# ZHANGKEON/DIS-YOLO

Hardware: AMD Instinct MI355X
Metric: train images/sec @576x576 bf16 (higher is better)
Workload: dtype bf16

## Files before the change

### dis-yolo_amd/csrc/conv_wgrad.hip

```cpp
#include "common.h"
#include "runtime.h"

namespace {

struct WgradParams {
  const bf16* x0;
  const bf16* x1;
  const bf16* dy;
  float* out;
  int B, H, W, C0, C1, Cin;
  int Ho, Wo, Cout, ldy;
  int ks, stride, pad_t, pad_l;
  int M, K;
  int steps_per_split, steps;
  int tilesK, tilesN;
  unsigned bytes0, bytes1, bytesy;
};

typedef __attribute__((address_space(3))) s16x4 lds_s16x4;
typedef int i32x4 __attribute__((ext_vector_type(4)));
constexpr unsigned OOB = 0x80000000u;

__device__ __forceinline__ int swz_u(int row, int u, int units) {
  const int h = (row & 3) | (((row >> 3) & 1) << 2);
// ... 93 lines not shown
#pragma unroll
  for (int j = 0; j < YI; ++j) {
    const int chunk = (j * NW + wave) * 64 + lane;
    const int row = chunk / YCH, pc = chunk % YCH;
    const int lc = swz_u(row, pc >> 1, YCH / 2) * 2 + (pc & 1);
    const int n = n0 + lc * 8;
    y_nok[j] = (row < 32) && (n < p.ldy);
    y_m[j] = step0 * 32 + row;
    y_off[j] = ((unsigned)y_m[j] * (unsigned)p.ldy + (unsigned)n) * 2u;
  }

  const bool mixed = (p.C1 > 0) && ((p.C0 & (BM - 1)) != 0);
  const bool blk_second = (p.C1 > 0) && (kt0 >= p.C0);
  auto issue_tile = [&](int stage) {
    const unsigned sbase = lds0 + stage * STB + wave * 1024;
#pragma unroll
    for (int j = 0; j < XI; ++j) {
      const int iy = x_yo[j] * p.stride - p.pad_t + x_kh[j];
      const int ix = x_xo[j] * p.stride - p.pad_l + x_kw[j];
      const bool ok = x_kok[j] && (x_b[j] < p.B) && ((unsigned)iy < (unsigned)p.H) && ((unsigned)ix < (unsigned)p.W);
      unsigned off;
      if (!x_second[j]) {
        off = (unsigned)(((x_b[j] * p.H + iy) * p.W + ix) * p.C0 + x_ci[j]) * 2u;
      } else {
        const int H1 = p.H >> 1, W1 = p.W >> 1;
        off = (unsigned)(((x_b[j] * H1 + (iy >> 1)) * W1 + (ix >> 1)) * p.C1 + x_ci[j]) * 2u;
      }
      if (!mixed) {
        if (blk_second) dma16(ok ? off : OOB, srd1, sbase + j * SLAB);
        else dma16(ok ? off : OOB, srd0, sbase + j * SLAB);
      } else {
        const void* src = ok ? (const void*)((const char*)(x_second[j] ? p.x1 : p.x0) + off) : (const void*)&g_zero16;
        dma16_flat(src, sbase + j * SLAB);
      }
      x_xo[j] += 32;
      while (x_xo[j] >= p.Wo) {
        x_xo[j] -= p.Wo;
        if (++x_yo[j] == p.Ho) {
          x_yo[j] = 0;
          ++x_b[j];
        }
      }
    }
#pragma unroll
    for (int j = 0; j < YI; ++j) {
      dma16((y_nok[j] && y_m[j] < p.M) ? y_off[j] : OOB, srdy, sbase + X_BYTES + j * SLAB);
      y_m[j] += 32;
      y_off[j] += 32u * (unsigned)p.ldy * 2u;
    }
  };

  f32x4 acc[MI][NI];
#pragma unroll
  for (int i = 0; i < MI; ++i)
#pragma unroll
    for (int j = 0; j < NI; ++j) acc[i][j] = f32x4{0.f, 0.f, 0.f, 0.f};

#pragma unroll
  for (int s = 0; s < PRE; ++s)
    if (s < nsteps) issue_tile(s);

  const int g = lane >> 4, li = lane & 15, q = li >> 2, pc = li & 3;
  for (int st = 0; st < nsteps; ++st) {
    if (PRE >= 1 && st + PRE - 1 < nsteps)
      wait_vmcnt<LPT*(PRE >= 1 ? PRE - 1 : 0)>();
    else
      wait_vmcnt<0>();
    __builtin_amdgcn_s_barrier();
    asm volatile("" ::: "memory");
    if (st + PRE < nsteps) issue_tile((st + PRE) % ST);
    const char* sX = smem + (st % ST) * STB;
    const char* sY = sX + X_BYTES;
    bf16x8 af[MI], bfr[NI];
    typedef short s16x8 __attribute__((ext_vector_type(8)));
    const int r0 = 8 * g + q, r1 = r0 + 4;
#pragma unroll
    for (int i = 0; i < MI; ++i) {
      const int u = (wm * WTM + i * 16) >> 4;
      const s16x4 lo = __builtin_amdgcn_ds_read_tr16_b64_v4i16(
          (lds_s16x4*)(sX + r0 * XP + swz_u(r0, u, XCH / 2) * 32 + pc * 8));
      const s16x4 hi = __builtin_amdgcn_ds_read_tr16_b64_v4i16(
          (lds_s16x4*)(sX + r1 * XP + swz_u(r1, u, XCH / 2) * 32 + pc * 8));
      const s16x8 v = {lo[0], lo[1], lo[2], lo[3], hi[0], hi[1], hi[2], hi[3]};
      af[i] = __builtin_bit_cast(bf16x8, v);
    }
#pragma unroll
    for (int j = 0; j < NI; ++j) {
      const int u = (wn * WTN + j * 16) >> 4;
      const s16x4 lo = __builtin_amdgcn_ds_read_tr16_b64_v4i16(
          (lds_s16x4*)(sY + r0 * YP + swz_u(r0, u, YCH / 2) * 32 + pc * 8));
      const s16x4 hi = __builtin_amdgcn_ds_read_tr16_b64_v4i16(
          (lds_s16x4*)(sY + r1 * YP + swz_u(r1, u, YCH / 2) * 32 + pc * 8));
      const s16x8 v = {lo[0], lo[1], lo[2], lo[3], hi[0], hi[1], hi[2], hi[3]};
      bfr[j] = __builtin_bit_cast(bf16x8, v);
    }
#pragma unroll
    for (int i = 0; i < MI; ++i)
#pragma unroll
      for (int j = 0; j < NI; ++j)
        acc[i][j] = __builtin_amdgcn_mfma_f32_16x16x32_bf16(af[i], bfr[j], acc[i][j], 0, 0, 0);
  }

  float* slab = p.out + (size_t)bsplit * p.K * p.Cout;
  __syncthreads();
  constexpr int ROWP = WTN * 4 + 16;
  constexpr int HALF = MI / 2 * 16;
  if constexpr (NW * HALF * ROWP <= ST * STB) {
    if ((p.Cout & 3) == 0) {
      char* sw = smem + wave * (HALF * ROWP);
      constexpr int CPR4 = WTN / 4, CH = HALF * CPR4;
#pragma unroll
      for (int h = 0; h < 2; ++h) {
#pragma unroll
        for (int i2 = 0; i2 < MI / 2; ++i2)
#pragma unroll
          for (int j = 0; j < NI; ++j)
#pragma unroll
            for (int r = 0; r < 4; ++r)
              *reinterpret_cast<float*>(sw + (i2 * 16 + g * 4 + r) * ROWP + (j * 16 + li) * 4) = acc[h * (MI / 2) + i2][j][r];
        __builtin_amdgcn_fence(__ATOMIC_RELEASE, "wavefront");
        __builtin_amdgcn_wave_barrier();
        __builtin_amdgcn_fence(__ATOMIC_ACQUIRE, "wavefront");
#pragma unroll
        for (int it = 0; it < (CH + 63) / 64; ++it) {
          const int idx = it * 64 + lane;
          const int row = idx / CPR4, ch = idx % CPR4;
          const int kk = kt0 + wm * WTM + h * HALF + row, n = n0 + wn * WTN + ch * 4;
          if (idx < CH && kk < p.K && n < p.Cout)
            *reinterpret_cast<float4*>(slab + (size_t)kk * p.Cout + n) =
                *reinterpret_cast<const float4*>(sw + row * ROWP + ch * 16);
        }
        __builtin_amdgcn_fence(__ATOMIC_RELEASE, "wavefront");
        __builtin_amdgcn_wave_barrier();
      }
      return;
    }
  }
#pragma unroll
  for (int i = 0; i < MI; ++i) {
#pragma unroll
    for (int j = 0; j < NI; ++j) {
      const int n = n0 + wn * WTN + j * 16 + li;
      if (n >= p.Cout) continue;
#pragma unroll
      for (int r = 0; r < 4; ++r) {
        const int kk = kt0 + wm * WTM + i * 16 + g * 4 + r;
        if (kk < p.K) slab[(size_t)kk * p.Cout + n] = acc[i][j][r];
      }
    }
  }
}


struct Wg3Params {
  const bf16* x;
  const bf16* dy;
  float* out;
  int B, H, W, Cin, Cout, ldy;
  int Ho, Wo;
  int P, Hp, frame, kbias;
  int a64, r64;
  int chunks, chunks_per_split;
  int tilesCi, tilesCo, tiles;
  int leadA, leadB;
  unsigned bytesx, bytesy;
  int debug;
};

struct PixState {
  int b, yy, xx;
};
__device__ __forceinline__ void pix_init(PixState& s, int Q, const Wg3Params& p) {
  const int Qn = Q + p.kbias * p.frame;
  const int bb = Qn / p.frame;
  const int rem = Qn - bb * p.frame;
  s.b = bb - p.kbias;
  s.yy = rem / p.P;
  s.xx = rem - s.yy * p.P;
}
__device__ __forceinline__ void pix_advance64(PixState& s, const Wg3Params& p) {
  s.xx += p.r64;
  s.yy += p.a64;
  if (s.xx >= p.P) {
    s.xx -= p.P;
    ++s.yy;
  }
  while (s.yy >= p.Hp) {
    s.yy -= p.Hp;
    ++s.b;
  }
}
__device__ __forceinline__ int pix_index(const PixState& s, const Wg3Params& p) {
  const bool ok = ((unsigned)s.b < (unsigned)p.B) && (s.yy >= 1) && (s.xx >= 1);
  return ok ? (s.b * p.H + s.yy - 1) * p.W + s.xx - 1 : -1;
}

__device__ __forceinline__ int pix_index_s2_in(const PixState& s, const Wg3Params& p) {
  const bool ok = ((unsigned)s.b < (unsigned)p.B) && (s.yy < p.Ho) && (s.xx < p.Wo);
  return ok ? (s.b * p.H + 2 * s.yy) * p.W + 2 * s.xx : -1;
}
__device__ __forceinline__ int pix_index_s2_out(const PixState& s, const Wg3Params& p) {
  const bool ok = ((unsigned)s.b < (unsigned)p.B) && (s.yy < p.Ho) && (s.xx < p.Wo);
  return ok ? (s.b * p.Ho + s.yy) * p.Wo + s.xx : -1;
}

template <int IMM>
__device__ __forceinline__ void dma16_imm(unsigned voff, i32x4 srd, unsigned lds_dst) {
  asm volatile("s_mov_b32 m0, %2\n\ts_nop 0\n\tbuffer_load_dwordx4 %0, %1, 0 offen offset:%3 lds"
               :
               : "v"(voff), "s"(srd), "s"(lds_dst - (unsigned)IMM), "n"(IMM)
               : "memory");
}

template <int CO_T, int R, int ST, int NW, int S2 = 0>
__global__ __launch_bounds__(NW * 64) void conv_wgrad3x3_kernel(Wg3Params p) {
  constexpr int NJ = CO_T / 32;
  constexpr int YD = CO_T / 32;
  constexpr int YDW = YD * 4 / NW;
  constexpr int TPW = NW == 8 ? 5 : 9;
  constexpr int YST = YD * 4096;
  constexpr int XRING = R * 4096;
  constexpr int XALLOC = XRING + 1024;
  constexpr int NR = S2 ? 4 : 1;
  constexpr int XTOT = NR * XALLOC;
  constexpr int PRE = ST - 1;
  constexpr int LPT0 = NR + YDW, LPT1 = YDW;
  static_assert(!S2 || NW == 4, "stride 2: the four-wave form only");
  static_assert((R & (R - 1)) == 0 && ST >= 2, "ring");

  extern __shared__ __attribute__((aligned(16))) char smem[];
  const unsigned lds0 = (unsigned)(size_t)(__attribute__((address_space(3))) char*)smem;
  const int tid = threadIdx.x, lane = tid & 63;
  const int wave = __builtin_amdgcn_readfirstlane(tid >> 6);
  const int wq = wave & 3, tg = wave >> 2;
  const int u = wq & 1, ch = wq >> 1;
  const int tap0 = tg * 5, ntaps = NW == 8 ? (tg ? 4 : 5) : 9;
  int lin;
  {
    const int nblk = gridDim.x, bid = blockIdx.x;
    const int q8 = nblk >> 3, r8 = nblk & 7, xcd = bid & 7, loc = bid >> 3;
    lin = (xcd < r8 ? xcd * (q8 + 1) : r8 * (q8 + 1) + (xcd - r8) * q8) + loc;
  }
  const int tile = lin % p.tiles, bsplit = lin / p.tiles;
  const int ci0 = (tile % p.tilesCi) * 32, co0 = (tile / p.tilesCi) * CO_T;
  const int c0 = bsplit * p.chunks_per_split;
  int c1 = c0 + p.chunks_per_split;
  if (c1 > p.chunks) c1 = p.chunks;
  const int nsteps = c1 - c0;

  const i32x4 srdx = make_srd(p.x, p.bytesx);
  const i32x4 srdy = make_srd(p.dy, p.bytesy);

  const int drow = wq * 16 + (lane >> 2), dpc = lane & 3;
  const int dlu = (dpc >> 1) ^ ((drow >> 2) & 1);
  const unsigned x_const = (unsigned)(ci0 + dlu * 16 + (dpc & 1) * 8) * 2u;
  const int y_n = co0 + (NW == 8 ? tg * 32 : 0) + dlu * 16 + (dpc & 1) * 8;
  const unsigned y_const = (unsigned)y_n * 2u;
  PixState xs, ys;
  pix_init(xs, (c0 - p.leadB) * 64 + drow, p);
  pix_init(ys, c0 * 64 + drow, p);
  const unsigned xrow_bytes = (unsigned)p.Cin * 2u, yrow_bytes = (unsigned)p.ldy * 2u;
  auto issue_x = [&](int c) {
    const unsigned slot = (unsigned)(c & (R - 1));
    if constexpr (S2) {
      const int pix = pix_index_s2_in(xs, p);
#pragma unroll
      for (int cls = 0; cls < 4; ++cls) {
        const unsigned voff = pix >= 0 ? (unsigned)(pix + (cls >> 1) * p.W + (cls & 1)) * xrow_bytes + x_const : OOB;
        if (wave == 0 && slot == 0) dma16(voff, srdx, lds0 + cls * XALLOC + XRING);
        dma16(voff, srdx, lds0 + cls * XALLOC + slot * 4096u + wq * 1024u);
      }
    } else {
      const int pix = pix_index(xs, p);
      const unsigned voff = pix >= 0 ? (unsigned)pix * xrow_bytes + x_const : OOB;
      if (tg == 0) {
        if (wave == 0 && slot == 0) dma16(voff, srdx, lds0 + XRING);
        dma16(voff, srdx, lds0 + slot * 4096u + wq * 1024u);
      }
    }
    pix_advance64(xs, p);
  };
  auto issue_y = [&](int stage) {
    const int pix = S2 ? pix_index_s2_out(ys, p) : pix_index(ys, p);
    const unsigned voff = pix >= 0 ? (unsigned)pix * yrow_bytes + y_const : OOB;
    const unsigned dst = lds0 + XTOT + stage * YST + (NW == 8 ? tg * 4096u : 0u) + wq * 1024u;
    dma16_imm<0>((y_n < p.ldy) ? voff : OOB, srdy, dst);
    if constexpr (NW == 4) {
      dma16_imm<64>((y_n + 32 < p.ldy) ? voff : OOB, srdy, dst + 4096u);
      if constexpr (YD == 4) {
        dma16_imm<128>((y_n + 64 < p.ldy) ? voff : OOB, srdy, dst + 8192u);
        dma16_imm<192>((y_n + 96 < p.ldy) ? voff : OOB, srdy, dst + 12288u);
      }
    } else if constexpr (YD == 4) {
      dma16_imm<128>((y_n + 64 < p.ldy) ? voff : OOB, srdy, dst + 8192u);
    }
    pix_advance64(ys, p);
  };

  const int g = lane >> 4, li = lane & 15, q = li >> 2, pc = li & 3;
  int E[TPW], EC[TPW];
#pragma unroll
  for (int i = 0; i < TPW; ++i) {
    const int tap = tap0 + i;
    const int kh = tap / 3, kw = tap % 3;
    const int rowc = (S2 ? (kh >> 1) * p.P + (kw >> 1) : (kh - 1) * p.P + (kw - 1)) + 4 * g + q;
    E[i] = rowc * 64 + ((u ^ ((rowc >> 2) & 1)) * 32) + pc * 8;
// ... 150 lines not shown
  const unsigned gbase = (unsigned)grp * 2u * F1_STB;
  const int g = lane >> 4, li = lane & 15, q = li >> 2, pc = li & 3;
  const i32x4 srdy = make_srd(dy, bytesy);
  const int drow = wave * 16 + (lane >> 2), dpc = lane & 3;
  const unsigned y_const = (unsigned)((((dpc >> 1) ^ ((drow >> 2) & 1)) * 16 + (dpc & 1) * 8) * 2);
  int e_x[2], e_c[2];
#pragma unroll
  for (int h = 0; h < 2; ++h) {
    const int e = tid + h * 256;
    e_x[h] = e / 3;
    e_c[h] = e - e_x[h] * 3;
  }
  float iv[3][2];
  auto unit_of = [&](int u, int& b, int& y, int& x0) {
    const int xb = u % units_x, r = u / units_x;
    y = r % H;
    b = r / H;
    x0 = xb * 128;
  };
  auto issue_dy = [&](int stage, int b, int y, int x0) {
#pragma unroll
    for (int s2 = 0; s2 < 2; ++s2) {
      const int x = x0 + s2 * 64 + drow;
      const unsigned voff = x < W ? (unsigned)((b * H + y) * W + x) * 64u + y_const : OOB;
      dma16(voff, srdy, lds0 + gbase + stage * F1_STB + F1_IMGB + s2 * 4096 + wave * 1024);
    }
  };
  auto load_img = [&](int b, int y, int x0) {
#pragma unroll
    for (int kh = 0; kh < 3; ++kh) {
      const int yy = y + kh - 1;
#pragma unroll
      for (int h = 0; h < 2; ++h) {
        const int x = x0 - 1 + e_x[h];
        const bool ok = (tid + h * 256 < 390) && ((unsigned)yy < (unsigned)H) && ((unsigned)x < (unsigned)W);
        iv[kh][h] = ok ? img[((size_t)(b * H + yy) * W + x) * 3 + e_c[h]] : 0.f;
      }
    }
  };
  auto write_img = [&](int stage) {
    char* base = smem + gbase + stage * F1_STB;
#pragma unroll
    for (int kh = 0; kh < 3; ++kh)
#pragma unroll
      for (int h = 0; h < 2; ++h) {
        if (tid + h * 256 >= 390) continue;
        const bf16 v = (bf16)iv[kh][h];
#pragma unroll
        for (int kw = 0; kw < 3; ++kw) {
          const int j = e_x[h] - kw;
          if ((unsigned)j < 128u) *reinterpret_cast<bf16*>(base + ((kh * 3 + kw) * 3 + e_c[h]) * F1_ROWB + j * 2) = v;
        }
      }
  };
  f32x4 acc[2][2];
#pragma unroll
  for (int f = 0; f < 2; ++f)
#pragma unroll
    for (int j = 0; j < 2; ++j) acc[f][j] = f32x4{0.f, 0.f, 0.f, 0.f};
  const int a_off = li * F1_ROWB + (32 * wave + 4 * g) * 2;
  const bool a1_ok = 16 + li < 27;
  const int brow = 4 * g + q;
  int Fy[2];
#pragma unroll
  for (int j = 0; j < 2; ++j)
    Fy[j] = F1_IMGB + (wave >> 1) * 4096 + (wave & 1) * 2048 + brow * 64 + ((j ^ ((brow >> 2) & 1)) * 32) + pc * 8;

  int u = blockIdx.x * 2 + grp;
  const int ustep = gridDim.x * 2;
  int stage = 0;
  if (u < nunits) {
    int b, y, x0;
    unit_of(u, b, y, x0);
    issue_dy(0, b, y, x0);
    load_img(b, y, x0);
    write_img(0);
  }
  wait_vmcnt<0>();
  __syncthreads();
  typedef short s16x8 __attribute__((ext_vector_type(8)));
  const int rounds = (nunits - (int)blockIdx.x * 2 + ustep - 1) / ustep;
  for (int it = 0; it < rounds; ++it, u += ustep) {
    const int un = u + ustep;
    const bool more = un < nunits;
    if (more) {
      int b, y, x0;
      unit_of(un, b, y, x0);
      issue_dy(stage ^ 1, b, y, x0);
      load_img(b, y, x0);
    }
    const char* sb = smem + gbase + stage * F1_STB;
    if (u < nunits) {
    bf16x8 af[2], bfr[2];
    {
      const uint2 lo = *reinterpret_cast<const uint2*>(sb + a_off), hi = *reinterpret_cast<const uint2*>(sb + a_off + 32);
      const uint4 v = {lo.x, lo.y, hi.x, hi.y};
      af[0] = __builtin_bit_cast(bf16x8, v);
      uint4 w = {0u, 0u, 0u, 0u};
      if (a1_ok) {
        const uint2 lo1 = *reinterpret_cast<const uint2*>(sb + a_off + 16 * F1_ROWB);
        const uint2 hi1 = *reinterpret_cast<const uint2*>(sb + a_off + 16 * F1_ROWB + 32);
        w = uint4{lo1.x, lo1.y, hi1.x, hi1.y};
      }
      af[1] = __builtin_bit_cast(bf16x8, w);
    }
#pragma unroll
    for (int j = 0; j < 2; ++j) {
      const char* a = sb + Fy[j];
      const s16x4 lo = __builtin_amdgcn_ds_read_tr16_b64_v4i16((lds_s16x4*)a);
      const s16x4 hi = __builtin_amdgcn_ds_read_tr16_b64_v4i16((lds_s16x4*)(a + 1024));
      const s16x8 v = {lo[0], lo[1], lo[2], lo[3], hi[0], hi[1], hi[2], hi[3]};
      bfr[j] = __builtin_bit_cast(bf16x8, v);
    }
#pragma unroll
    for (int f = 0; f < 2; ++f)
#pragma unroll
      for (int j = 0; j < 2; ++j) acc[f][j] = __builtin_amdgcn_mfma_f32_16x16x32_bf16(af[f], bfr[j], acc[f][j], 0, 0, 0);
    }
    if (more) write_img(stage ^ 1);
    wait_vmcnt<0>();
    __syncthreads();
    stage ^= 1;
  }
  float* red = reinterpret_cast<float*>(smem);
  __syncthreads();
#pragma unroll
  for (int f = 0; f < 2; ++f)
#pragma unroll
    for (int j = 0; j < 2; ++j)
#pragma unroll
      for (int r = 0; r < 4; ++r) red[((grp * 4 + wave) * 32 + 16 * f + 4 * g + r) * 32 + 16 * j + li] = acc[f][j][r];
  __syncthreads();
  float* slab = slabs + (size_t)blockIdx.x * 27 * 32;
  for (int o = threadIdx.x; o < 27 * 32; o += 512)
    slab[o] = ((red[o] + red[1024 + o]) + (red[2048 + o] + red[3072 + o])) + ((red[4096 + o] + red[5120 + o]) + (red[6144 + o] + red[7168 + o]));
}

void plan(const disyolo_conv_desc* d, int* bn, int* splits, int* steps_per_split, int* steps) {
  const int M = d->B * d->Ho * d->Wo;
  const int K = d->ksize * d->ksize * (d->C0 + d->C1);
  *bn = d->Cout > 64 ? 128 : (d->Cout > 32 ? 64 : 32);
  const int tiles = ceil_div(K, 128) * ceil_div(d->Cout, *bn);
  *steps = ceil_div(M, 32);
  const int target = 256, min_steps = 16;
  int s = target / tiles;
  if (s < 1) s = 1;
  const int max_s = ceil_div(*steps, min_steps);
  if (s > max_s) s = max_s;
  if (s < 1) s = 1;
  *steps_per_split = ceil_div(*steps, s);
  *splits = ceil_div(*steps, *steps_per_split);
}


constexpr int WG3_ST = 3;
struct Plan3 {
  int co_t, R, splits, cps, chunks, tilesCi, tilesCo, leadA, leadB, s2;
  size_t lds;
};
bool plan3(const disyolo_conv_desc* d, int opts, Plan3* q) {
  const int target = 192;
  if (opts & DISYOLO_WGRAD_IM2COL) return false;
  if (d->ksize != 3 || d->C1 != 0 || d->in_div != 1 || d->C0 % 32 || d->Cout % 4 || d->Cout < 32) return false;
  q->s2 = 0;
  if (d->stride == 2) {
    if (d->pad_t != 0 || d->pad_l != 0 || (d->H & 1) || (d->W & 1) || d->Ho * 2 != d->H || d->Wo * 2 != d->W) return false;
    q->s2 = 1;
  } else if (d->stride != 1 || d->pad_t != 1 || d->pad_l != 1 || d->Ho != d->H || d->Wo != d->W) {
    return false;
  }
  const int P = d->Wo + 1, Hp = d->Ho + 1;
  q->co_t = d->Cout > 64 ? 128 : 64;
  if (q->co_t == 128) {
    const int t128 = (d->C0 / 32) * ceil_div(d->Cout, 128);
    if ((target + t128 / 2) / t128 == 2) q->co_t = 64;
  }
  q->leadB = q->s2 ? 0 : ceil_div(P + 1, 64);
  q->leadA = 1 + P / 64;
  if (q->s2) q->co_t = 64;
  const int need = (WG3_ST - 1) + q->leadA + q->leadB + 1;
  q->R = need <= 8 ? 8 : (need <= 16 ? 16 : 32);
  for (;;) {
    q->lds = (size_t)(q->s2 ? 4 : 1) * ((size_t)q->R * 4096 + 1024) + (size_t)WG3_ST * 64 * (size_t)q->co_t * 2;
    if (need <= 32 && q->lds <= 160 * 1024) break;
    if (q->co_t == 128) { q->co_t = 64; continue; }
    return false;
  }
  q->chunks = ceil_div((int64_t)d->B * Hp * P, 64);
  q->tilesCi = d->C0 / 32;
  q->tilesCo = ceil_div(d->Cout, q->co_t);
  const int tiles = q->tilesCi * q->tilesCo;
  int s = (target + tiles / 2) / tiles;
  const int max_s = q->chunks / 4 > 1 ? q->chunks / 4 : 1;
  if (s > max_s) s = max_s;
  if (s < 1) s = 1;
  q->cps = ceil_div(q->chunks, s);
  q->splits = ceil_div(q->chunks, q->cps);
  return true;
}
template <int CO_T, int R>
int launch3(const Wg3Params& p, const Plan3& q, hipStream_t s) {
  static bool attr_done = false;
  auto fn = conv_wgrad3x3_kernel<CO_T, R, WG3_ST, 4>;
  if (!attr_done) {
    if (hipFuncSetAttribute((const void*)fn, hipFuncAttributeMaxDynamicSharedMemorySize, 160 * 1024) != hipSuccess) {
      (void)hipGetLastError();
    }
    attr_done = true;
  }
  hipLaunchKernelGGL(fn, dim3(q.tilesCi * q.tilesCo * q.splits), dim3(256), q.lds, s, p);
  return 0;
}
int launch3_s2(const Wg3Params& p, const Plan3& q, hipStream_t s) {
  static bool attr_done = false;
  auto fn = conv_wgrad3x3_kernel<64, 8, WG3_ST, 4, 1>;
  if (!attr_done) {
    if (hipFuncSetAttribute((const void*)fn, hipFuncAttributeMaxDynamicSharedMemorySize, 160 * 1024) != hipSuccess) (void)hipGetLastError();
    attr_done = true;
  }
  hipLaunchKernelGGL(fn, dim3(q.tilesCi * q.tilesCo * q.splits), dim3(256), q.lds, s, p);
  return 0;
}

}

extern "C" size_t disyolo_conv2d_wgrad_workspace(const disyolo_conv_desc* d, int opts) {
  if (!d) return 0;
  int bn, splits, sps, steps;
  plan(d, &bn, &splits, &sps, &steps);
  Plan3 q;
  if (plan3(d, opts, &q)) splits = q.splits;
  const size_t K = (size_t)d->ksize * d->ksize * (d->C0 + d->C1);
  return (size_t)splits * K * d->Cout * sizeof(float);
}

extern "C" int disyolo_conv2d_wgrad_plan(const disyolo_conv_desc* d, int opts, int* kind, int* tile_n, int* ring, int* splits) {
  if (!d || !kind || !tile_n || !ring || !splits) return DISYOLO_E_ARG;
  Plan3 q;
  if (plan3(d, opts, &q)) {
    *kind = 1; *tile_n = q.co_t; *ring = q.R; *splits = q.splits;
    return DISYOLO_OK;
  }
  int bn, sp, sps, steps;
  plan(d, &bn, &sp, &sps, &steps);
  *kind = 0; *tile_n = bn; *ring = 0; *splits = sp;
  return DISYOLO_OK;
}

extern "C" int disyolo_conv2d_wgrad(const disyolo_conv_desc* d, const void* dy, int dy_ld, float* dw, void* workspace,
                                    size_t workspace_bytes, int opts, void* stream) {
  DY_REQUIRE(d && dy && dw, "wgrad: null pointer");
  DY_REQUIRE(d->ksize == 1 || d->ksize == 3, "wgrad: ksize");
  DY_REQUIRE(d->C0 > 0 && d->C0 % 8 == 0 && d->C1 % 8 == 0, "wgrad: channels must be multiples of 8");
  DY_REQUIRE(d->C1 == 0 || (d->ksize == 1 && d->stride == 1 && d->x1), "wgrad: bad fused-concat layer");
  DY_REQUIRE(dy_ld >= d->Cout && dy_ld % 8 == 0, "wgrad: dy_ld must be >= Cout and a multiple of 8");
  DY_REQUIRE(d->in_div == 1, "wgrad: in_div must be 1");
  DY_REQUIRE((int64_t)d->B * d->H * d->W * d->C0 * 2 < (1LL << 31) && (int64_t)d->B * d->Ho * d->Wo * dy_ld * 2 < (1LL << 31),
             "wgrad: a source tensor exceeds the 2 GiB the 32-bit gather offsets address");
  DY_REQUIRE((opts & ~(DISYOLO_WGRAD_IM2COL | DISYOLO_WGRAD_PARTIAL_ONLY | DISYOLO_WGRAD_REDUCE_ONLY | DISYOLO_WGRAD_STAGES_MASK)) == 0,
             "wgrad: unknown opts bits");
  if (!workspace || workspace_bytes < disyolo_conv2d_wgrad_workspace(d, opts)) {
    disyolo_set_error("wgrad: workspace too small");
    return DISYOLO_E_WORKSPACE;
  }
  {
    const disyolo_conv_desc c = *d;
    DY_RECORD_OR_RUN([=](void* s) { return disyolo_conv2d_wgrad(&c, dy, dy_ld, dw, workspace, workspace_bytes, opts, s); });
  }
  Plan3 q3;
  if (plan3(d, opts, &q3)) {
    Wg3Params p;
    p.x = (const bf16*)d->x0;
    p.dy = (const bf16*)dy;
    p.B = d->B; p.H = d->H; p.W = d->W; p.Cin = d->C0; p.Cout = d->Cout; p.ldy = dy_ld;
    p.Ho = d->Ho; p.Wo = d->Wo;
    p.P = d->Wo + 1; p.Hp = d->Ho + 1; p.frame = p.Hp * p.P;
    p.kbias = q3.s2 ? 0 : ceil_div((q3.leadB + 1) * 64, p.frame);
    p.a64 = 64 / p.P; p.r64 = 64 % p.P;
    p.chunks = q3.chunks; p.chunks_per_split = q3.cps;
    p.tilesCi = q3.tilesCi; p.tilesCo = q3.tilesCo; p.tiles = q3.tilesCi * q3.tilesCo;
    p.leadA = q3.leadA; p.leadB = q3.leadB;
    p.bytesx = (unsigned)((size_t)d->B * d->H * d->W * d->C0 * 2);
    p.bytesy = (unsigned)((size_t)d->B * d->Ho * d->Wo * dy_ld * 2);
    p.out = q3.splits == 1 ? dw : (float*)workspace;
    p.debug = 0;
    hipStream_t s = (hipStream_t)stream;
    if (opts & DISYOLO_WGRAD_REDUCE_ONLY) goto reduce3;
    if (q3.s2) {
      launch3_s2(p, q3, s);
    } else if (q3.co_t == 128) {
      if (q3.R == 8) launch3<128, 8>(p, q3, s);
      else if (q3.R == 16) launch3<128, 16>(p, q3, s);
      else launch3<128, 32>(p, q3, s);
    } else {
      if (q3.R == 8) launch3<64, 8>(p, q3, s);
      else if (q3.R == 16) launch3<64, 16>(p, q3, s);
      else launch3<64, 32>(p, q3, s);
    }
    DY_CHECK_LAUNCH();
  reduce3:
    if (q3.splits > 1 && !(opts & DISYOLO_WGRAD_PARTIAL_ONLY)) {
      const int64_t n = (int64_t)9 * p.Cin * p.Cout;
      hipLaunchKernelGGL(slab_reduce_kernel, dim3(ceil_div(n, 64)), dim3(256), 0, s, (const float*)workspace, dw, n,
                         q3.splits);
      DY_CHECK_LAUNCH();
    }
    return DISYOLO_OK;
  }
  WgradParams p;
  p.x0 = (const bf16*)d->x0;
  p.x1 = (const bf16*)d->x1;
  p.dy = (const bf16*)dy;
  p.B = d->B; p.H = d->H; p.W = d->W; p.C0 = d->C0; p.C1 = d->C1; p.Cin = d->C0 + d->C1;
  p.Ho = d->Ho; p.Wo = d->Wo; p.Cout = d->Cout; p.ldy = dy_ld;
  p.ks = d->ksize; p.stride = d->stride; p.pad_t = d->pad_t; p.pad_l = d->pad_l;
  p.M = d->B * d->Ho * d->Wo;
  p.K = d->ksize * d->ksize * p.Cin;
  p.bytes0 = (unsigned)((size_t)d->B * d->H * d->W * d->C0 * 2);
  p.bytes1 = (unsigned)((size_t)d->B * (d->H / 2) * (d->W / 2) * d->C1 * 2);
  p.bytesy = (unsigned)((size_t)p.M * dy_ld * 2);
  int bn, splits;
  plan(d, &bn, &splits, &p.steps_per_split, &p.steps);
  p.out = splits == 1 ? dw : (float*)workspace;
  hipStream_t s = (hipStream_t)stream;
  p.tilesK = ceil_div(p.K, 128);
  p.tilesN = ceil_div(p.Cout, bn);
  dim3 grid(p.tilesK * p.tilesN * splits);
  const int sto = (opts & DISYOLO_WGRAD_STAGES_MASK) >> 4;
  const int st = sto ? sto + 1 : 3;
  if (opts & DISYOLO_WGRAD_REDUCE_ONLY) goto reduce1;
#define DY_WG(BNV, YB)                                                                                   \
  if (st == 2) hipLaunchKernelGGL((conv_wgrad_kernel<BNV, 2>), grid, dim3(256), 2 * (8192 + YB), s, p);      \
  else if (st == 3) hipLaunchKernelGGL((conv_wgrad_kernel<BNV, 3>), grid, dim3(256), 3 * (8192 + YB), s, p); \
  else hipLaunchKernelGGL((conv_wgrad_kernel<BNV, 4>), grid, dim3(256), 4 * (8192 + YB), s, p);
  if (bn == 128) { DY_WG(128, 8192) }
  else if (bn == 64) { DY_WG(64, 4096) }
  else { DY_WG(32, 4096) }
#undef DY_WG
  DY_CHECK_LAUNCH();
reduce1:
  if (splits > 1 && !(opts & DISYOLO_WGRAD_PARTIAL_ONLY)) {
    const int64_t n = (int64_t)p.K * p.Cout;
    hipLaunchKernelGGL(slab_reduce_kernel, dim3(ceil_div(n, 64)), dim3(256), 0, s, (const float*)workspace, dw, n,
                       splits);
    DY_CHECK_LAUNCH();
  }
  return DISYOLO_OK;
}

static int first_wgrad_blocks(int B, int H, int W) {
  const int64_t pairs = ((int64_t)B * H * ceil_div(W, 128) + 1) / 2;
  return (int)(pairs < 512 ? pairs : 512);
}

extern "C" size_t disyolo_conv_first_wgrad_workspace(int B, int H, int W, int Cout) {
  const int64_t M = (int64_t)B * H * W;
  const int blocks = ceil_div(M, 1024);
  const size_t direct = (size_t)blocks * 27 * Cout * sizeof(float);
  const size_t mfma = (size_t)first_wgrad_blocks(B, H, W) * 27 * 32 * sizeof(float);
  return direct > mfma ? direct : mfma;
}

extern "C" int disyolo_conv_first_wgrad(const float* images, const void* dy, float* dw, int B, int H, int W, int Cout,
                                        void* workspace, size_t workspace_bytes, void* stream) {
  DY_REQUIRE(images && dy && dw && B > 0 && H > 0 && W > 0 && Cout > 0 && 27 * Cout <= 1024, "first_wgrad: bad args");
  if (!workspace || workspace_bytes < disyolo_conv_first_wgrad_workspace(B, H, W, Cout)) {
    disyolo_set_error("first_wgrad: workspace too small");
    return DISYOLO_E_WORKSPACE;
  }
  DY_RECORD_OR_RUN([=](void* s) { return disyolo_conv_first_wgrad(images, dy, dw, B, H, W, Cout, workspace, workspace_bytes, s); });
  const int64_t M = (int64_t)B * H * W;
  hipStream_t s = (hipStream_t)stream;
  const int64_t n = 27 * Cout;
  if (Cout == 32 && M * 64 < (1LL << 31)) {
    const int units_x = ceil_div(W, 128);
    const int nunits = B * H * units_x;
    const int blocks = first_wgrad_blocks(B, H, W);
    hipLaunchKernelGGL(conv_first_wgrad_mfma_kernel, dim3(blocks), dim3(512), 4 * F1_STB, s, images, (const bf16*)dy,
                       (float*)workspace, B, H, W, units_x, nunits, (unsigned)(M * 64));
    DY_CHECK_LAUNCH();
    hipLaunchKernelGGL(slab_reduce_kernel, dim3(ceil_div(n, 64)), dim3(256), 0, s, (const float*)workspace, dw, n, blocks);
    DY_CHECK_LAUNCH();
    return DISYOLO_OK;
  }
  const int blocks = ceil_div(M, 1024);
  hipLaunchKernelGGL(conv_first_wgrad_kernel, dim3(blocks), dim3(1024), 0, s, images, (const bf16*)dy,
                     (float*)workspace, B, H, W, Cout, 1024);
  DY_CHECK_LAUNCH();
  hipLaunchKernelGGL(slab_reduce_kernel, dim3(ceil_div(n, 64)), dim3(256), 0, s, (const float*)workspace, dw, n,
                     blocks);
  DY_CHECK_LAUNCH();
  return DISYOLO_OK;
}
```

### dis-yolo_amd/lib.py

```python
from __future__ import annotations

import ctypes as C
import os
from typing import Optional

import numpy as np
import torch

_HERE = os.path.dirname(os.path.abspath(__file__))
LIB_PATH = os.environ.get("DISYOLO_LIB", os.path.join(_HERE, "libdisyolo_hip.so"))

GRAD_LD = 32
MAX_BOXES = 256
MAX_DET = 256
ROI_MAX = 16
ROI_W = 12
ROI_CAP = 512
K_MAPS = (3, 5, 7)
MASK_STRIDES = (1, 2, 4)
NMS_MODES = {"per_class": 0, "agnostic": 1, "none": 2}


def roi_w(k: int) -> int:
    return 2 * (k + 1) + 4
# ... 613 lines not shown
                   residual_scale: float = 0.0) -> None:
    if TIMER is not None:
        name = "conv_fp8_kernel<%d,%d,3>" % (128 if d.Cout > 64 else (64 if d.Cout > 32 else 32), 64 if d.C0 % 64 == 0 else 32)
        TIMER.run(name, conv_flops(d), lambda: _check(load().disyolo_conv2d_fp8_fwd(
            C.byref(d), _p(w8), _p(escale), _p(eshift), _p(residual8), residual_scale, _p(y8), out_scale, _p(y16), _stream()),
            "conv2d_fp8_fwd"))
        return
    _check(load().disyolo_conv2d_fp8_fwd(C.byref(d), _p(w8), _p(escale), _p(eshift), _p(residual8), residual_scale, _p(y8),
                                         out_scale, _p(y16), _stream()), "conv2d_fp8_fwd")


def conv_first_fwd_fp8(images, w_hwio, scale, shift, y8, out_scale: float, alpha=0.1) -> None:
    _need(images, torch.float32, "images")
    _need(y8, torch.uint8, "y8")
    B, H, W, _ = images.shape
    _check(load().disyolo_conv_first_fwd_fp8(_p(images), _p(w_hwio), _p(scale), _p(shift), _p(y8), out_scale, B, H, W,
                                             y8.shape[-1], alpha, _stream()), "conv_first_fwd_fp8")


def quant_fp8(x, y8, scale: float) -> None:
    if x.dtype not in (torch.bfloat16, torch.float32) or not x.is_contiguous():
        raise DisyoloError("quant_fp8: x must be contiguous bf16 or f32")
    _check(load().disyolo_quant_fp8(_p(x), int(x.dtype == torch.float32), _p(y8), x.numel(), scale, _stream()), "quant_fp8")


def dequant_fp8(x8, y, scale: float) -> None:
    _need(y, torch.float32, "y")
    _check(load().disyolo_dequant_fp8(_p(x8), _p(y), x8.numel(), scale, _stream()), "dequant_fp8")


def pack_weights_fp8(w_hwio, w8, ksize, cin, cout, scale: float) -> None:
    _check(load().disyolo_pack_weights_fp8(_p(w_hwio), _p(w8), ksize, cin, cout, scale, _stream()), "pack_weights_fp8")


def conv12_fused_ok(B: int, H: int, W: int) -> bool:
    return load().disyolo_conv12_fused_ok(B, H, W) == 1


def conv12_fused_fwd(images, w1_hwio, scale1, shift1, w2_packed, scale2, shift2, y, alpha=0.1) -> None:
    _need(images, torch.float32, "images")
    _need(y, torch.bfloat16, "y")
    B, H, W, _ = images.shape
    _need_shape(y, (B, H // 2, W // 2, 64), "conv12_fused_fwd: y")
    fn = lambda: _check(load().disyolo_conv12_fused_fwd(_p(images), _p(w1_hwio), _p(scale1), _p(shift1), _p(w2_packed), _p(scale2),
                                                        _p(shift2), _p(y), B, H, W, alpha, _stream()), "conv12_fused_fwd")
    if TIMER is not None:
        flops = 2.0 * B * H * W * 32 * 27 + 2.0 * B * (H // 2) * (W // 2) * 64 * 288
        TIMER.run("conv12_fused_kernel", flops, fn, float(B * H * W * 12 + B * (H // 2) * (W // 2) * 128))
        return
    fn()


def block32_fused_ok(B: int, H: int, W: int, C0: int, C1: int, post: int) -> bool:
    return load().disyolo_block32_fused_ok(B, H, W, C0, C1, post) == 1


def block32_fused_fwd(x0, x1, wA, scaleA, shiftA, wB, scaleB, shiftB, y, post=0, wC=None, biasC=None, alpha=0.1) -> None:
    _need(x0, torch.bfloat16, "x0")
    _need(y, torch.bfloat16 if post == 0 else torch.float32, "y")
    B, H, W, C0 = x0.shape
    C1 = 0 if x1 is None else x1.shape[-1]
    if x1 is not None:
        _need(x1, torch.bfloat16, "x1")
        _need_shape(x1, (B, H // 2, W // 2, C1), "block32_fused_fwd: x1")
    _need_shape(y, (B, H, W, {0: 64, 1: 9, 2: 25, 3: 49}[post]), "block32_fused_fwd: y")
    fn = lambda: _check(load().disyolo_block32_fused_fwd(_p(x0), _p(x1), C0, C1, _p(wA), _p(scaleA), _p(shiftA), _p(wB), _p(scaleB),
                                                         _p(shiftB), post, _p(wC), _p(biasC), _p(y), B, H, W, alpha, _stream()),
                        "block32_fused_fwd")
    if TIMER is not None:
        M = B * H * W
        flops = 2.0 * M * (32 * (C0 + C1) + 64 * 288 + (64 * 9 if post else 0))
        nbytes = M * C0 * 2 + (M // 4) * C1 * 2 + (M * 36 if post else M * 128)
        TIMER.run("block32_kernel<%d,%d>" % (C0 + C1, post), flops, fn, float(nbytes))
        return
    fn()


def dgrad_s2_quad_ok(B: int, Hdy: int, Wdy: int, Cdy: int, C: int) -> bool:
    return load().disyolo_dgrad_s2_quad_ok(B, Hdy, Wdy, Cdy, C) == 1


def pack_quad(w_hwio, wq) -> None:
    _need(w_hwio, torch.float32, "w")
    _need(wq, torch.bfloat16, "wq")
    C_, Cdy = w_hwio.shape[2], w_hwio.shape[3]
    _check(load().disyolo_pack_quad(_p(w_hwio), _p(wq), C_, Cdy, _stream()), "pack_quad")


def dgrad_s2_quad(dy, wq, dx, accumulate: bool = False) -> None:
    _need(dy, torch.bfloat16, "dy")
    _need(dx, torch.bfloat16, "dx")
    B, H, W, Cdy = dy.shape
    C_ = dx.shape[-1]
    fn = lambda: _check(load().disyolo_dgrad_s2_quad(_p(dy), _p(wq), _p(dx), _p(dx) if accumulate else None, B, H, W, Cdy, C_,
                                                      _stream()), "dgrad_s2_quad")
    if TIMER is not None:
        TIMER.run("conv_igemm_kernel<192,128,4,2,64,2,3,1>", 2.0 * B * H * W * 4 * C_ * 4 * Cdy, fn,
                  float(B * H * W * (Cdy + 4 * C_) * 2))
        return
    fn()


def block64_fused_ok(B: int, H: int, W: int, C0: int) -> bool:
    return load().disyolo_block64_fused_ok(B, H, W, C0) == 1


def block64_fused_fwd(x, wA, scaleA, shiftA, wB, scaleB, shiftB, y, alpha=0.1) -> None:
    _need(x, torch.bfloat16, "x")
    _need(y, torch.bfloat16, "y")
    B, H, W, C0 = x.shape
    _need_shape(y, (B, H, W, C0), "block64_fused_fwd: y")
    fn = lambda: _check(load().disyolo_block64_fused_fwd(_p(x), _p(wA), _p(scaleA), _p(shiftA), _p(wB), _p(scaleB), _p(shiftB), _p(y),
                                                         B, H, W, C0, alpha, _stream()), "block64_fused_fwd")
    if TIMER is not None:
        M = B * H * W
        TIMER.run("block64_kernel", 2.0 * M * (64 * 128 + 128 * 576), fn, float(M * 512))
        return
    fn()


def conv_first_fwd(images, w_hwio, scale, shift, y, alpha=0.1) -> None:
    _need(images, torch.float32, "images")
    _need(y, torch.bfloat16, "y")
    B, H, W, _ = images.shape
    _check(load().disyolo_conv_first_fwd(_p(images), _p(w_hwio), _p(scale), _p(shift), _p(y), B, H, W, y.shape[-1],
                                         alpha, _stream()), "conv_first_fwd")


WGRAD_IM2COL, WGRAD_PARTIAL_ONLY, WGRAD_REDUCE_ONLY = 1, 2, 4


def wgrad_stages(n: int) -> int:
    if not 2 <= int(n) <= 4:
        raise DisyoloError("wgrad_stages: 2..4 pipeline stages (got %r)" % (n,))
    return (int(n) - 1) << 4


def conv2d_wgrad_workspace(d: ConvDesc, opts: int = 0) -> int:
    return load().disyolo_conv2d_wgrad_workspace(C.byref(d), opts)


def conv2d_wgrad(d: ConvDesc, dy, dy_ld: int, dw, ws: Workspace, opts: int = 0) -> None:
    need = conv2d_wgrad_workspace(d, opts)
    buf = ws.get(need)

    def call(o):
        _check(load().disyolo_conv2d_wgrad(C.byref(d), _p(dy), dy_ld, _p(dw), _p(buf), buf.numel(), o, _stream()),
               "conv2d_wgrad")
    if TIMER is not None and not (opts & (WGRAD_PARTIAL_ONLY | WGRAD_REDUCE_ONLY)):
        kind, tn, ring, splits = conv2d_wgrad_plan(d, opts)
        name = ("conv_wgrad3x3_kernel<%d,%d,3,4,0>" % (tn, ring)) if kind == 1 else ("conv_wgrad_kernel<%d,3>" % tn)
        if kind == 1 and d.stride == 2:
            name = "conv_wgrad3x3_kernel<64,8,3,4,1>"
        TIMER.run(name, conv_flops(d), lambda: call(opts | WGRAD_PARTIAL_ONLY))
        if splits > 1:
            TIMER.run("slab_reduce_kernel", 0.0, lambda: call(opts | WGRAD_REDUCE_ONLY))
        return
    call(opts)


def conv2d_wgrad_plan(d: ConvDesc, opts: int = 0):
    v = [C.c_int(0) for _ in range(4)]
    _check(load().disyolo_conv2d_wgrad_plan(C.byref(d), opts, *[C.byref(x) for x in v]), "conv2d_wgrad_plan")
    return tuple(x.value for x in v)


def conv_first_wgrad(images, dy, dw, ws: Workspace) -> None:
    B, H, W, _ = images.shape
    cout = dy.shape[-1]
    need = load().disyolo_conv_first_wgrad_workspace(B, H, W, cout)
    buf = ws.get(need)
    _check(load().disyolo_conv_first_wgrad(_p(images), _p(dy), _p(dw), B, H, W, cout, _p(buf), buf.numel(), _stream()),
           "conv_first_wgrad")


def copy2d_f32(src, dst, rows, cols, src_ld, dst_ld) -> None:
    _check(load().disyolo_copy2d_f32(_p(src), _p(dst), rows, cols, src_ld, dst_ld, _stream()), "copy2d_f32")


def pack_weights(w_hwio, w_fwd, w_dgrad, ksize, cin, cout, cout_pad=0) -> None:
    _check(load().disyolo_pack_weights(_p(w_hwio), _p(w_fwd), _p(w_dgrad), ksize, cin, cout, max(cout_pad, cout),
                                       _stream()), "pack_weights")


class PackJob(C.Structure):
    _fields_ = [("w_hwio", C.c_void_p), ("w_fwd", C.c_void_p), ("w_dgrad", C.c_void_p),
                ("ksize", C.c_int32), ("Cin", C.c_int32), ("Cout", C.c_int32), ("cout_pad", C.c_int32)]


class PackTable:

    def __init__(self, jobs, device):
        n = len(jobs)
        arr = (PackJob * n)()
        for i, (w, wf, wd, k, cin, cout, pad) in enumerate(jobs):
            arr[i] = PackJob(_p(w), _p(wf), _p(wd), k, cin, cout, pad)
        nbytes = load().disyolo_pack_table_bytes(n)
        host = (C.c_char * nbytes)()
        blocks = C.c_int(0)
        _check(load().disyolo_pack_table_build(arr, n, host, C.byref(blocks)), "pack_table_build")
        self.n, self.blocks = n, blocks.value
        self.dev = torch.frombuffer(bytearray(bytes(host)), dtype=torch.uint8).to(device)
        self.keep = jobs

    def run(self) -> None:
        _check(load().disyolo_pack_all(_p(self.dev), self.n, self.blocks, _stream()), "pack_all")


def bn_finalize(stats, rows, C_, count, gamma, beta, mm, mv, decay, eps, scale, shift, mean, rstd) -> None:
    _check(load().disyolo_bn_finalize(_p(stats), rows, C_, count, _p(gamma), _p(beta), _p(mm), _p(mv), decay, eps,
                                      _p(scale), _p(shift), _p(mean), _p(rstd), _stream()), "bn_finalize")


def colstats_rows(rows, C_) -> int:
    r = load().disyolo_colstats_rows(rows, C_)
    if r < 0:
        raise DisyoloError("colstats_rows: bad shape")
    return r


def colstats(x, stats, rows, C_) -> None:
    _check(load().disyolo_colstats(_p(x), _p(stats), rows, C_, _stream()), "colstats")


def bn_act_bwd_partials(dy, x, scale, shift, mean, rstd, dx, dgamma, dbeta, rows, C_, partials, part_rows,
                        ws: Workspace, alpha=0.1, shortcut_grad=None, shortcut_accumulate=False) -> None:
    _need(partials, torch.float32, "partials")
    if partials.numel() < part_rows * C_ * 2:
        raise DisyoloError("bn_act_bwd_partials: partials smaller than part_rows x C x 2")
    buf = ws.get(load().disyolo_bn_act_bwd_partials_workspace(C_))
    _check(load().disyolo_bn_act_bwd_partials(_p(dy), _p(x), _p(scale), _p(shift), _p(mean), _p(rstd), _p(dx), _p(dgamma),
                                              _p(dbeta), rows, C_, alpha, _p(partials), part_rows, _p(shortcut_grad),
                                              int(shortcut_accumulate), _p(buf), buf.numel(), _stream()), "bn_act_bwd_partials")


def bn_partial_sums(partials, rows, C_, sums) -> None:
    _need(sums, torch.float64, "sums")
    _check(load().disyolo_bn_partial_sums(_p(partials), rows, C_, _p(sums), _stream()), "bn_partial_sums")


def bn_finalize_sums(sums, C_, count, gamma, beta, mm, mv, decay, eps, scale, shift, mean, rstd) -> None:
    _need(sums, torch.float64, "sums")
    _check(load().disyolo_bn_finalize_sums(_p(sums), C_, count, _p(gamma), _p(beta), _p(mm), _p(mv), decay, eps, _p(scale),
                                           _p(shift), _p(mean), _p(rstd), _stream()), "bn_finalize_sums")


def bn_bwd_reduce(dy, x, scale, shift, mean, rstd, rows, C_, sums, ws: Workspace, alpha=0.1) -> None:
    _need(sums, torch.float64, "sums")
    buf = ws.get(load().disyolo_bn_bwd_reduce_rows(rows, C_) * C_ * 2 * 4)
    _check(load().disyolo_bn_bwd_reduce(_p(dy), _p(x), _p(scale), _p(shift), _p(mean), _p(rstd), rows, C_, alpha, _p(sums),
                                        _p(buf), buf.numel(), _stream()), "bn_bwd_reduce")


def bn_bwd_apply_sums(dy, x, scale, shift, mean, rstd, local_sums, global_sums, count, dx, dgamma, dbeta, rows, C_,
                      ws: Workspace, alpha=0.1, shortcut_grad=None, shortcut_accumulate=False) -> None:
    buf = ws.get(2 * C_ * 4)
    _check(load().disyolo_bn_bwd_apply_sums(_p(dy), _p(x), _p(scale), _p(shift), _p(mean), _p(rstd), _p(local_sums),
                                            _p(global_sums), count, _p(dx), _p(dgamma), _p(dbeta), rows, C_, alpha,
                                            _p(shortcut_grad), int(shortcut_accumulate), _p(buf), buf.numel(), _stream()),
           "bn_bwd_apply_sums")


def bn_fold(gamma, beta, mm, mv, eps, scale, shift) -> None:
    _check(load().disyolo_bn_fold(_p(gamma), _p(beta), _p(mm), _p(mv), eps, _p(scale), _p(shift), gamma.numel(),
                                  _stream()), "bn_fold")


def bn_act_fwd(x, scale, shift, residual, y, rows, C_, alpha=0.1) -> None:
    _check(load().disyolo_bn_act_fwd(_p(x), _p(scale), _p(shift), _p(residual), _p(y), rows, C_, alpha, _stream()),
           "bn_act_fwd")


def bn_act_bwd(dy, x, scale, shift, mean, rstd, dx, dgamma, dbeta, rows, C_, ws: Workspace, alpha=0.1,
               shortcut_grad=None, shortcut_accumulate=False) -> None:
    need = load().disyolo_bn_act_bwd_workspace(rows, C_)
    buf = ws.get(need)
    _check(load().disyolo_bn_act_bwd(_p(dy), _p(x), _p(scale), _p(shift), _p(mean), _p(rstd), _p(dx), _p(dgamma),
                                     _p(dbeta), rows, C_, alpha, _p(shortcut_grad), int(shortcut_accumulate), _p(buf),
                                     buf.numel(), _stream()), "bn_act_bwd")


def bn_frozen_bwd(dy, x, scale, shift, dx, rows, C_, alpha=0.1, shortcut_grad=None, shortcut_accumulate=False) -> None:
    _check(load().disyolo_bn_frozen_bwd(_p(dy), _p(x), _p(scale), _p(shift), _p(dx), rows, C_, alpha, _p(shortcut_grad),
                                        int(shortcut_accumulate), _stream()), "bn_frozen_bwd")


def mask_paste(masks, rects, classids, image_h: int, image_w: int, full_masks, merged) -> None:
    n = int(rects.shape[0])
    if n:
        _need(masks, torch.float32, "masks")
        _need(rects, torch.int32, "rects")
        _need(classids, torch.int32, "classids")
    mh, mw = (int(masks.shape[-2]), int(masks.shape[-1])) if n else (1, 1)
    _check(load().disyolo_mask_paste_hw(_p(masks) if n else None, n, mh, mw, _p(rects) if n else None,
                                        _p(classids) if n else None, image_h, image_w, _p(full_masks), _p(merged), _stream()),
           "mask_paste")


PASTE_JOB = np.dtype([("masks", np.uint64), ("rects", np.uint64), ("classids", np.uint64), ("gt", np.uint64), ("gt_class", np.uint64),
                      ("merged", np.uint64), ("true_map", np.uint64), ("counts", np.uint64), ("n", np.int32), ("ng", np.int32),
                      ("image_h", np.int32), ("image_w", np.int32), ("block0", np.int32), ("reserved", np.int32)])
assert PASTE_JOB.itemsize == 88


def paste_job_plan(jobs, wide: bool = False) -> int:
    if jobs.dtype != PASTE_JOB or not jobs.flags["C_CONTIGUOUS"] or jobs.ndim != 1:
# ... 872 lines not shown
```

Measured before the change: 2199.

## Add multi-stage streaming wgrad kernel for small 1x1 convolutions

Adds a dedicated weight-gradient kernel for 1x1 stride-1 convolutions with at most 256 input and 64 output channels and large spatial extent. A persistent grid of up to 256 blocks walks several split ranges each and keeps all K rows resident per block. It uses a deep multi-stage LDS ring of buffer DMA loads, with magic-number division for the fused upsampled concat input. The aim is to hide global load latency and cut per-block overhead on these bandwidth-bound layers, at the cost of large LDS use and lower occupancy.

```diff
diff --git a/dis-yolo_amd/csrc/conv_wgrad.hip b/dis-yolo_amd/csrc/conv_wgrad.hip
--- a/dis-yolo_amd/csrc/conv_wgrad.hip
+++ b/dis-yolo_amd/csrc/conv_wgrad.hip
@@ -269,6 +269,187 @@
 }
 
 
+struct WgsParams {
+  const bf16* x0;
+  const bf16* x1;
+  const bf16* dy;
+  float* out;
+  int H, W, C0, C1, Cout, ldy;
+  int M, K, np0;
+  int steps_per_split, steps, splits;
+  unsigned bytes0, bytes1, bytesy;
+  unsigned magic_hw, magic_w;
+};
+
+__device__ __forceinline__ void divmod_magic(unsigned m, unsigned d, unsigned magic, unsigned& q, unsigned& r) {
+  q = __umulhi(m, magic);
+  r = m - q * d;
+  if (r >= d) {
+    ++q;
+    r -= d;
+  }
+}
+
+constexpr int wgs_sp(int np) { return np <= 2 ? 128 : 64; }
+constexpr int wgs_stage_bytes(int np, int bn) { return wgs_sp(np) * (np * 128 + bn * 2); }
+constexpr int wgs_stages(int np, int bn) {
+  const int n = 144 * 1024 / wgs_stage_bytes(np, bn);
+  return n > 5 ? 5 : n;
+}
+
+template <int NP, int BN>
+__global__ __launch_bounds__(256) void conv_wgrad_stream_kernel(WgsParams p) {
+  constexpr int SP = wgs_sp(NP), GPS = SP / 32;
+  constexpr int MI = NP, NI = BN / 16;
+  constexpr int PANELB = SP * 128, YP = BN * 2;
+  constexpr int XB = NP * PANELB, YB = SP * YP, STB = XB + YB;
+  constexpr int NS = wgs_stages(NP, BN), PRE = NS - 1;
+  constexpr int XI = XB / 4096, YI = YB / 4096, LPT = XI + YI;
+  static_assert(XB % 4096 == 0 && YB % 4096 == 0 && NS >= 3 && LPT * (PRE - 1) < 64, "stage shape");
+
+  extern __shared__ __attribute__((aligned(16))) char smem[];
+  const unsigned lds0 = (unsigned)(size_t)(__attribute__((address_space(3))) char*)smem;
+  const int tid = threadIdx.x, lane = tid & 63;
+  const int wave = __builtin_amdgcn_readfirstlane(tid >> 6);
+
+  const int nb = gridDim.x, bid = blockIdx.x;
+  const int s0 = (int)((int64_t)bid * p.splits / nb), s1 = (int)((int64_t)(bid + 1) * p.splits / nb);
+  const int G0 = s0 * p.steps_per_split;
+  int G1 = s1 * p.steps_per_split;
+  if (G1 > p.steps) G1 = p.steps;
+  const int T = (G1 - G0 + GPS - 1) / GPS;
+  int mlim = G1 * 32;
+  if (mlim > p.M) mlim = p.M;
+
+  const i32x4 srd0 = make_srd(p.x0, p.bytes0);
+  const i32x4 srd1 = make_srd(p.x1 ? (const void*)p.x1 : (const void*)p.x0, p.x1 ? p.bytes1 : 0u);
+  const i32x4 srdy = make_srd(p.dy, p.bytesy);
+
+  const int xrow = lane >> 3;
+  const int xkey = ((lane >> 4) & 1) | ((wave & 1) << 1);
+  const int xcol = (((((lane & 7) >> 1) ^ xkey) << 1) | (lane & 1)) * 8;
+  const int yrow = BN == 64 ? xrow : lane >> 2;
+  const int ycol = BN == 64 ? xcol : ((((((lane & 3) >> 1) ^ ((lane >> 5) & 1)) << 1) | (lane & 1)) * 8);
+  const int H1 = p.H >> 1, W1 = p.W >> 1, hw = p.H * p.W;
+
+  auto issue_stage = [&](int t, int slot) {
+    const int m0 = (G0 + t * GPS) * 32;
+    const unsigned sbase = lds0 + slot * STB + wave * 1024;
+#pragma unroll
+    for (int j = 0; j < XI; ++j) {
+      constexpr int PPW = SP / 32;
+      const int panel = j / PPW;
+      const int m = m0 + ((j % PPW) * 4 + wave) * 8 + xrow;
+      const bool mok = m < mlim;
+      if (panel < p.np0) {
+        const int c = panel * 64 + xcol;
+        dma16((mok && c < p.C0) ? ((unsigned)m * (unsigned)p.C0 + (unsigned)c) * 2u : OOB, srd0, sbase + j * 4096);
+      } else {
+        const int c = (panel - p.np0) * 64 + xcol;
+        const int mm = mok ? m : 0;
+        unsigned b, rem, y, x;
+        divmod_magic((unsigned)mm, (unsigned)hw, p.magic_hw, b, rem);
+        divmod_magic(rem, (unsigned)p.W, p.magic_w, y, x);
+        const unsigned off = (unsigned)(((b * H1 + (y >> 1)) * W1 + (x >> 1)) * p.C1 + c) * 2u;
+        dma16((mok && c < p.C1) ? off : OOB, srd1, sbase + j * 4096);
+      }
+    }
+#pragma unroll
+    for (int j = 0; j < YI; ++j) {
+      const int m = m0 + (j * 4 + wave) * (BN == 64 ? 8 : 16) + yrow;
+      dma16((m < mlim && ycol < p.ldy) ? ((unsigned)m * (unsigned)p.ldy + (unsigned)ycol) * 2u : OOB, srdy,
+            sbase + XB + j * 4096);
+    }
+  };
+
+  const int g = lane >> 4, li = lane & 15, q = li >> 2, pc = li & 3;
+  const int rkey = ((q >> 1) & 1) | ((g & 1) << 1);
+  int aoff[MI];
+  bool kf_ok[MI];
+#pragma unroll
+  for (int i = 0; i < MI; ++i) {
+    const int kf = i * 4 + wave;
+    kf_ok[i] = kf * 16 < p.K;
+    const int kcol = kf * 16 + 4 * pc;
+    const bool second = p.C1 > 0 && kcol >= p.C0;
+    const int kk = second ? kcol - p.C0 : kcol;
+    const int pan = (second ? p.np0 : 0) + (kk >> 6), c = kk & 63;
+    aoff[i] = pan * PANELB + (8 * g + q) * 128 + (((c >> 4) ^ rkey) << 5) + (c & 15) * 2;
+  }
+  int boff[NI];
+#pragma unroll
+  for (int j = 0; j < NI; ++j) boff[j] = XB + (8 * g + q) * YP + ((j ^ (NI == 4 ? rkey : (g & 1))) << 5) + pc * 8;
+
+  f32x4 acc[MI][NI];
+#pragma unroll
+  for (int i = 0; i < MI; ++i)
+#pragma unroll
+    for (int j = 0; j < NI; ++j) acc[i][j] = f32x4{0.f, 0.f, 0.f, 0.f};
+
+  typedef short s16x8 __attribute__((ext_vector_type(8)));
+  int split = s0, bnd = G0 + p.steps_per_split;
+  int cslot = 0, islot = 0;
+  for (int tt = 0; tt < T + PRE; ++tt) {
+    const int t = tt - PRE;
+    if (t >= 0) {
+      if (tt <= T)
+        wait_vmcnt<LPT*(PRE - 1)>();
+      else
+        wait_vmcnt<0>();
+      __builtin_amdgcn_s_barrier();
+      asm volatile("" ::: "memory");
+    }
+    if (tt < T) issue_stage(tt, islot);
+    if (++islot == NS) islot = 0;
+    if (t < 0) continue;
+    const char* sb = smem + cslot * STB;
+    if (++cslot == NS) cslot = 0;
+#pragma unroll
+    for (int gi = 0; gi < GPS; ++gi) {
+      const int grp = G0 + t * GPS + gi;
+      if (grp >= G1) break;
+      bf16x8 bfr[NI];
+#pragma unroll
+      for (int j = 0; j < NI; ++j) {
+        const char* a = sb + boff[j] + gi * 32 * YP;
+        const s16x4 lo = __builtin_amdgcn_ds_read_tr16_b64_v4i16((lds_s16x4*)a);
+        const s16x4 hi = __builtin_amdgcn_ds_read_tr16_b64_v4i16((lds_s16x4*)(a + 4 * YP));
+        const s16x8 v = {lo[0], lo[1], lo[2], lo[3], hi[0], hi[1], hi[2], hi[3]};
+        bfr[j] = __builtin_bit_cast(bf16x8, v);
+      }
+#pragma unroll
+      for (int i = 0; i < MI; ++i) {
+        if (!kf_ok[i]) continue;
+        const char* a = sb + aoff[i] + gi * 32 * 128;
+        const s16x4 lo = __builtin_amdgcn_ds_read_tr16_b64_v4i16((lds_s16x4*)a);
+        const s16x4 hi = __builtin_amdgcn_ds_read_tr16_b64_v4i16((lds_s16x4*)(a + 4 * 128));
+        const s16x8 v = {lo[0], lo[1], lo[2], lo[3], hi[0], hi[1], hi[2], hi[3]};
+        const bf16x8 af = __builtin_bit_cast(bf16x8, v);
+#pragma unroll
+        for (int j = 0; j < NI; ++j) acc[i][j] = __builtin_amdgcn_mfma_f32_16x16x32_bf16(af, bfr[j], acc[i][j], 0, 0, 0);
+      }
+      if (grp + 1 == bnd || grp + 1 == G1) {
+        float* slab = p.out + (size_t)split * p.K * p.Cout;
+#pragma unroll
+        for (int i = 0; i < MI; ++i)
+#pragma unroll
+          for (int j = 0; j < NI; ++j) {
+            const int n = j * 16 + li;
+#pragma unroll
+            for (int r = 0; r < 4; ++r) {
+              const int kk = (i * 4 + wave) * 16 + g * 4 + r;
+              if (kk < p.K && n < p.Cout) slab[(size_t)kk * p.Cout + n] = acc[i][j][r];
+              acc[i][j][r] = 0.f;
+            }
+          }
+        ++split;
+        bnd += p.steps_per_split;
+      }
+    }
+  }
+}
+
+
 struct Wg3Params {
   const bf16* x;
   const bf16* dy;
@@ -725,6 +906,35 @@
   *splits = ceil_div(*steps, *steps_per_split);
 }
 
+constexpr int WGS_MIN_M = 4096;
+constexpr int WGS_BLOCKS = 256;
+struct PlanS {
+  int np0, np, bn, splits, steps_per_split, steps, blocks;
+};
+bool plan_stream(const disyolo_conv_desc* d, int opts, PlanS* q) {
+  if (opts & DISYOLO_WGRAD_IM2COL) return false;
+  if (d->ksize != 1 || d->stride != 1 || d->in_div != 1 || d->pad_t != 0 || d->pad_l != 0) return false;
+  if (d->Ho != d->H || d->Wo != d->W || d->C0 <= 0 || d->C1 < 0) return false;
+  if (d->C0 + d->C1 > 256 || d->Cout > 64 || d->Cout < 1) return false;
+  if ((int64_t)d->B * d->Ho * d->Wo < WGS_MIN_M) return false;
+  q->np0 = ceil_div(d->C0, 64);
+  q->np = q->np0 + ceil_div(d->C1, 64);
+  if (q->np > 4) return false;
+  plan(d, &q->bn, &q->splits, &q->steps_per_split, &q->steps);
+  q->blocks = q->splits < WGS_BLOCKS ? q->splits : WGS_BLOCKS;
+  return true;
+}
+template <int NP, int BN>
+void launch_stream(const WgsParams& p, const PlanS& q, hipStream_t s) {
+  static bool attr_done = false;
+  auto fn = conv_wgrad_stream_kernel<NP, BN>;
+  constexpr int lds = wgs_stages(NP, BN) * wgs_stage_bytes(NP, BN);
+  if (!attr_done) {
+    if (hipFuncSetAttribute((const void*)fn, hipFuncAttributeMaxDynamicSharedMemorySize, lds) != hipSuccess) (void)hipGetLastError();
+    attr_done = true;
+  }
+  hipLaunchKernelGGL(fn, dim3(q.blocks), dim3(256), lds, s, p);
+}
 
 constexpr int WG3_ST = 3;
 struct Plan3 {
@@ -812,6 +1022,11 @@
   Plan3 q;
   if (plan3(d, opts, &q)) {
     *kind = 1; *tile_n = q.co_t; *ring = q.R; *splits = q.splits;
+    return DISYOLO_OK;
+  }
+  PlanS qs;
+  if (plan_stream(d, opts, &qs)) {
+    *kind = 2; *tile_n = qs.bn; *ring = qs.np; *splits = qs.splits;
     return DISYOLO_OK;
   }
   int bn, sp, sps, steps;
@@ -876,6 +1091,43 @@
       const int64_t n = (int64_t)9 * p.Cin * p.Cout;
       hipLaunchKernelGGL(slab_reduce_kernel, dim3(ceil_div(n, 64)), dim3(256), 0, s, (const float*)workspace, dw, n,
                          q3.splits);
+      DY_CHECK_LAUNCH();
+    }
+    return DISYOLO_OK;
+  }
+  PlanS qs;
+  if (plan_stream(d, opts, &qs)) {
+    WgsParams p;
+    p.x0 = (const bf16*)d->x0;
+    p.x1 = (const bf16*)d->x1;
+    p.dy = (const bf16*)dy;
+    p.H = d->H; p.W = d->W; p.C0 = d->C0; p.C1 = d->C1; p.Cout = d->Cout; p.ldy = dy_ld;
+    p.M = d->B * d->Ho * d->Wo;
+    p.K = d->C0 + d->C1;
+    p.np0 = qs.np0;
+    p.steps_per_split = qs.steps_per_split; p.steps = qs.steps; p.splits = qs.splits;
+    p.bytes0 = (unsigned)((size_t)p.M * d->C0 * 2);
+    p.bytes1 = (unsigned)((size_t)d->B * (d->H / 2) * (d->W / 2) * d->C1 * 2);
+    p.bytesy = (unsigned)((size_t)p.M * dy_ld * 2);
+    auto magic = [](int64_t dd) { const uint64_t v = (1ull << 32) / (uint64_t)dd; return (unsigned)(v > 0xffffffffull ? 0xffffffffull : v); };
+    p.magic_hw = magic((int64_t)d->H * d->W);
+    p.magic_w = magic(d->W);
+    p.out = qs.splits == 1 ? dw : (float*)workspace;
+    hipStream_t s = (hipStream_t)stream;
+    if (!(opts & DISYOLO_WGRAD_REDUCE_ONLY)) {
+#define DY_WGS(NPV)                                          \
+  if (qs.bn == 64) launch_stream<NPV, 64>(p, qs, s);         \
+  else launch_stream<NPV, 32>(p, qs, s);
+      if (qs.np == 1) { DY_WGS(1) }
+      else if (qs.np == 2) { DY_WGS(2) }
+      else if (qs.np == 3) { DY_WGS(3) }
+      else { DY_WGS(4) }
+#undef DY_WGS
+      DY_CHECK_LAUNCH();
+    }
+    if (qs.splits > 1 && !(opts & DISYOLO_WGRAD_PARTIAL_ONLY)) {
+      const int64_t n = (int64_t)p.K * p.Cout;
+      hipLaunchKernelGGL(slab_reduce_kernel, dim3(ceil_div(n, 64)), dim3(256), 0, s, (const float*)workspace, dw, n, qs.splits);
       DY_CHECK_LAUNCH();
     }
     return DISYOLO_OK;
diff --git a/dis-yolo_amd/lib.py b/dis-yolo_amd/lib.py
--- a/dis-yolo_amd/lib.py
+++ b/dis-yolo_amd/lib.py
@@ -789,6 +789,8 @@
         name = ("conv_wgrad3x3_kernel<%d,%d,3,4,0>" % (tn, ring)) if kind == 1 else ("conv_wgrad_kernel<%d,3>" % tn)
         if kind == 1 and d.stride == 2:
             name = "conv_wgrad3x3_kernel<64,8,3,4,1>"
+        if kind == 2:
+            name = "conv_wgrad_stream_kernel<%d,%d>" % (ring, tn)
         TIMER.run(name, conv_flops(d), lambda: call(opts | WGRAD_PARTIAL_ONLY))
         if splits > 1:
             TIMER.run("slab_reduce_kernel", 0.0, lambda: call(opts | WGRAD_REDUCE_ONLY))
```

Result: no change. 2206, median of 4 (+0.4%).
